# matteociccozzi/LayoutDiT

Hardware: AMD Instinct MI355X
Metric: images/sec ViT-B/16 224px bs=64 fwd (higher is better)
Workload: dtype f32; 1 GPU; ViT-base/16 224x224 bs=64 f32 forward, taps [4, 6, 8, 12] (BASELINE.json configs[1]); images_per_gpu=64, global_batch=64, parallelism=dp1: batch-sharded replicas, no data-path collective, weights=synthetic seed 0, images=synthetic doc-like pages, seed 1234, rank0_placement=128 CPUs: NUMA node 1 of GPU 0000:a4:00.0

## Files before the change

layoutdit_amd/csrc/attention_f32.hip:

```cpp
#include "ldit_common.h"

#ifdef LDIT_GEMM_STAMPS
__device__ unsigned long long *g_attn32_stamps = nullptr;
#define A32_STAMP(var) const unsigned long long var = __builtin_amdgcn_s_memtime()
#else
#define A32_STAMP(var)
#endif

namespace ldit {

namespace {

constexpr int KSTR = 68;
constexpr int VSTR = 64;

template <int KT, int NW>
__global__ void __launch_bounds__(NW * 64, NW == 4 ? 2 : NW / 4) attention_f32(const float *__restrict__ Q, const float *__restrict__ K,
                                                     const float *__restrict__ V, float *__restrict__ O, int N, int H,
                                                     int ldq, int ldk, int ldv, int ldo, float scale, int nqg)
{
    constexpr int KROWS = KT * 32;
    extern __shared__ __attribute__((aligned(16))) char smem[];
    float *Ks = reinterpret_cast<float *>(smem);
    float *Vs = Ks + KROWS * KSTR;

    const int tid = threadIdx.x, lane = tid & 63;
    const int wave = __builtin_amdgcn_readfirstlane(tid >> 6);
    const int li = lane & 31, lh = lane >> 5;
    const int bid = blockIdx.x;
    const int qg = bid % nqg, bh = bid / nqg, head = bh % H, b = bh / H;
    const int qt = qg * NW + wave;
    const bool active = qt * 32 < N;
    const size_t tok0 = (size_t)b * N;
#ifdef LDIT_GEMM_STAMPS
    unsigned long long ph[4] = {0, 0, 0, 0};
#endif
    A32_STAMP(t_begin);

    float q[32];
    {
        int qrow = qt * 32 + li;
        qrow = qrow < N ? qrow : N - 1;
        const f32x4 *qp = reinterpret_cast<const f32x4 *>(Q + (tok0 + qrow) * ldq + head * 64 + 32 * lh);
#pragma unroll
        for (int u = 0; u < 8; ++u) {
            const f32x4 t = qp[u];
            q[4 * u + 0] = t[0]; q[4 * u + 1] = t[1]; q[4 * u + 2] = t[2]; q[4 * u + 3] = t[3];
        }
    }

    f32x16 o[2];
#pragma unroll
    for (int e = 0; e < 16; ++e) { o[0][e] = 0.0f; o[1][e] = 0.0f; }
    float m_run = -INFINITY, l_run = 0.0f;

    for (int c0 = 0; c0 < N; c0 += KROWS) {
        const int nkeys = (N - c0) < KROWS ? (N - c0) : KROWS;
        const int ktiles = (nkeys + 31) >> 5;
        A32_STAMP(t0);
        if (c0) __syncthreads();
        {
            constexpr int PER = (32 * 16) / (NW * 64) > 0 ? (32 * 16) / (NW * 64) : 1;
            static_assert((32 * 16) % (NW * 64) == 0, "a key tile must split evenly over the threads");
            constexpr int BATCH = 4;
#pragma unroll
            for (int e = 0; e < PER; ++e)
#pragma unroll
                for (int k0 = 0; k0 < KT; k0 += BATCH) {
                    f32x4 kv[BATCH], vv[BATCH];
#pragma unroll
                    for (int i = 0; i < BATCH; ++i) {
                        const int kt = k0 + i, u = kt * 512 + e * NW * 64 + tid, row = u >> 4, c4 = (u & 15) * 4;
                        kv[i] = f32x4{0.f, 0.f, 0.f, 0.f};
                        vv[i] = f32x4{0.f, 0.f, 0.f, 0.f};
                        if (kt < KT && kt < ktiles && row < nkeys) {
                            kv[i] = *reinterpret_cast<const f32x4 *>(K + (tok0 + c0 + row) * ldk + head * 64 + c4);
                            vv[i] = *reinterpret_cast<const f32x4 *>(V + (tok0 + c0 + row) * ldv + head * 64 + c4);
                        }
                    }
#pragma unroll
                    for (int i = 0; i < BATCH; ++i) {
                        const int kt = k0 + i, u = kt * 512 + e * NW * 64 + tid, row = u >> 4, c4 = (u & 15) * 4;
                        if (kt < KT && kt < ktiles) {
                            *reinterpret_cast<f32x4 *>(Ks + row * KSTR + c4) = kv[i];
                            *reinterpret_cast<f32x4 *>(Vs + row * VSTR + c4) = vv[i];
                        }
                    }
                }
        }
        __syncthreads();
        if (!active) continue;
        A32_STAMP(t1);

        f32x16 s[KT];
#pragma unroll
        for (int kt = 0; kt < KT; ++kt) {
#pragma unroll
            for (int e = 0; e < 16; ++e) s[kt][e] = 0.0f;
            if (kt < ktiles) {
                const float *kr = Ks + (kt * 32 + li) * KSTR + 32 * lh;
#pragma unroll
                for (int u = 0; u < 8; ++u) {
                    const f32x4 kf = *reinterpret_cast<const f32x4 *>(kr + 4 * u);
#pragma unroll
                    for (int e = 0; e < 4; ++e)
                        s[kt] = __builtin_amdgcn_mfma_f32_32x32x2f32(kf[e], q[4 * u + e], s[kt], 0, 0, 0);
                }
            }
        }
#ifdef LDIT_GEMM_STAMPS
        asm volatile("s_nop 0" ::"v"(s[0][0]), "v"(s[KT - 1][0]));
#endif
        A32_STAMP(t2);
        float mx = -INFINITY;
#pragma unroll
        for (int kt = 0; kt < KT; ++kt) {
            if (kt < ktiles) {
                const bool partial = (kt + 1) * 32 > nkeys;
#pragma unroll
                for (int r = 0; r < 16; ++r) {
                    float v = s[kt][r] * scale;
                    if (partial && (kt * 32 + 8 * (r >> 2) + 4 * lh + (r & 3)) >= nkeys) v = -INFINITY;
                    s[kt][r] = v;
                    mx = fmaxf(mx, v);
                }
            }
        }
        mx = fmaxf(mx, __shfl_xor(mx, 32, 64));
        const float m_new = fmaxf(m_run, mx);
        const float alpha = __expf(m_run - m_new);
        m_run = m_new;
        float lsum = 0.0f;
#pragma unroll
        for (int kt = 0; kt < KT; ++kt) {
            if (kt < ktiles) {
#pragma unroll
                for (int r = 0; r < 16; ++r) {
                    const float pv = __expf(s[kt][r] - m_new);
                    s[kt][r] = pv;
                    lsum += pv;
                }
            }
        }
        l_run = l_run * alpha + lsum;
        if (c0) {
#pragma unroll
            for (int e = 0; e < 16; ++e) { o[0][e] *= alpha; o[1][e] *= alpha; }
        }
        A32_STAMP(t3);
#pragma unroll
        for (int kt = 0; kt < KT; ++kt) {
            if (kt < ktiles) {
                const int left = nkeys - kt * 32;
#pragma unroll
                for (int r = 0; r < 16; ++r) {
                    if (8 * (r >> 2) + (r & 3) >= left) continue;
                    const float *vr = Vs + (kt * 32 + 8 * (r >> 2) + 4 * lh + (r & 3)) * VSTR + li;
                    o[0] = __builtin_amdgcn_mfma_f32_32x32x2f32(vr[0], s[kt][r], o[0], 0, 0, 0);
                    o[1] = __builtin_amdgcn_mfma_f32_32x32x2f32(vr[32], s[kt][r], o[1], 0, 0, 0);
                }
            }
        }
#ifdef LDIT_GEMM_STAMPS
        asm volatile("s_nop 0" ::"v"(o[0][0]), "v"(o[1][0]));
        ph[0] += t1 - t0 + (c0 ? 0 : t0 - t_begin); ph[1] += t2 - t1; ph[2] += t3 - t2; ph[3] += __builtin_amdgcn_s_memtime() - t3;
#endif
    }

    if (!active) return;
#ifdef LDIT_GEMM_STAMPS
    if (g_attn32_stamps && wave == 0 && lane == 0) {
        unsigned long long *d = g_attn32_stamps + (size_t)blockIdx.x * 6;
        d[0] = ph[0]; d[1] = ph[1]; d[2] = ph[2]; d[3] = ph[3]; d[5] = __builtin_amdgcn_s_memtime() - t_begin;
    }
#endif
    const float l = l_run + __shfl_xor(l_run, 32, 64);
    const float inv = 1.0f / l;
    const int qrow = qt * 32 + li;
    if (qrow < N) {
        float *op = O + (tok0 + qrow) * ldo + head * 64 + 4 * lh;
#pragma unroll
        for (int dt = 0; dt < 2; ++dt)
#pragma unroll
            for (int g = 0; g < 4; ++g) {
                f32x4 t = {o[dt][4 * g + 0] * inv, o[dt][4 * g + 1] * inv, o[dt][4 * g + 2] * inv, o[dt][4 * g + 3] * inv};
                *reinterpret_cast<f32x4 *>(op + dt * 32 + 8 * g) = t;
            }
    }
}

}

int launch_attention(const float *Q, const float *K, const float *V, float *O, int B, int N, int H, int D, int ldq,
                     int ldk, int ldv, int ldo, float scale, hipStream_t stream)
{
    if (B <= 0 || N <= 0 || H <= 0) return fail(LDIT_EINVAL, "attention: empty problem");
    if (D != 64) return fail(LDIT_EUNSUPPORTED, "attention: head_dim=%d, only 64 is implemented", D);
    if (!Q || !K || !V || !O) return fail(LDIT_EINVAL, "attention: null operand");
    if ((ldq | ldk | ldv | ldo) & 3) return fail(LDIT_EINVAL, "attention: row strides must be multiples of 4 floats");
    if (!aligned16(Q) || !aligned16(K) || !aligned16(V) || !aligned16(O)) return fail(LDIT_EINVAL, "attention: operands must be 16-byte aligned");
    constexpr int KT = 7;
    constexpr int lds = KT * 32 * (KSTR + VSTR) * 4;
    const int nqt = (N + 31) / 32;
    auto go = [&](auto kern, int nw, std::atomic<unsigned long long> &attr_done) -> int {
        if (int rc = ensure_dynamic_lds(reinterpret_cast<const void *>(kern), lds, attr_done)) return rc;
        const int nqg = (nqt + nw - 1) / nw;
        hipLaunchKernelGGL(kern, dim3((unsigned)(B * H * nqg)), dim3(nw * 64), lds, stream, Q, K, V, O, N, H, ldq, ldk, ldv, ldo,
                           scale, nqg);
        LDIT_HIP_CHECK(hipGetLastError());
        return LDIT_OK;
    };
    static std::atomic<unsigned long long> set8{0}, set4{0};
    const long wgs8 = (long)B * H * ((nqt + 7) / 8);
    if (wgs8 <= 128 && nqt > 4) { if (int rc = go(attention_f32<KT, 4>, 4, set4)) return rc; }
    else if (int rc = go(attention_f32<KT, 8>, 8, set8)) return rc;
    LDIT_HIP_CHECK(hipGetLastError());
    return LDIT_OK;
}

}

#ifdef LDIT_GEMM_STAMPS
extern "C" int ldit_dbg_set_attn32_stamps(void *buf)
{
    unsigned long long *p = static_cast<unsigned long long *>(buf);
    return hipMemcpyToSymbol(HIP_SYMBOL(g_attn32_stamps), &p, sizeof(p)) == hipSuccess ? 0 : -3;
}
#endif
```

Baseline: 3432 images/sec.

## Use direct global-to-LDS loads and a persistent pipelined walk in f32 attention

Replaces the register-staged K/V copy into LDS with global_load_lds_dwordx4 direct-to-LDS DMA, using an XOR-swizzled K layout in place of the padded stride. When the whole sequence fits one key chunk (N <= 224, which holds for ViT-B/16's 197 tokens), it launches a persistent grid of one workgroup per CU. Each workgroup walks (image, head, query-group) items and prefetches the next item's K and Q while computing the current S and PV. The goal is to hide global load latency and cut VGPR traffic and launch tail. The cost is inline asm that manipulates m0, more complex barrier ordering, and fewer resident workgroups per CU.

```diff
diff --git a/layoutdit_amd/csrc/attention_f32.hip b/layoutdit_amd/csrc/attention_f32.hip
--- a/layoutdit_amd/csrc/attention_f32.hip
+++ b/layoutdit_amd/csrc/attention_f32.hip
@@ -11,34 +11,83 @@
 
 namespace {
 
-constexpr int KSTR = 68;
-constexpr int VSTR = 64;
-
-template <int KT, int NW>
+constexpr int ROWB = 256;
+
+__device__ __forceinline__ void glds16_sbase(const void *ubase, unsigned voff_bytes, unsigned lds_dst)
+{
+    unsigned keep;
+    asm volatile("s_mov_b32 %0, m0\n\ts_mov_b32 m0, %3\n\ts_nop 0\n\tglobal_load_lds_dwordx4 %1, %2\n\ts_mov_b32 m0, %0"
+                 : "=&s"(keep)
+                 : "v"(voff_bytes), "s"(ubase), "s"(lds_dst)
+                 : "memory");
+}
+
+__device__ __forceinline__ void dma_wait_and_barrier()
+{
+    asm volatile("s_waitcnt vmcnt(0)" ::: "memory");
+    __builtin_amdgcn_s_barrier();
+    asm volatile("" ::: "memory");
+}
+
+template <int KT, int NW, bool WALK>
 __global__ void __launch_bounds__(NW * 64, NW == 4 ? 2 : NW / 4) attention_f32(const float *__restrict__ Q, const float *__restrict__ K,
                                                      const float *__restrict__ V, float *__restrict__ O, int N, int H,
-                                                     int ldq, int ldk, int ldv, int ldo, float scale, int nqg)
-{
-    constexpr int KROWS = KT * 32;
+                                                     int ldq, int ldk, int ldv, int ldo, float scale, int nqg, int nitems)
+{
+    constexpr int KROWS = KT * 32, HALF = KROWS * ROWB;
+    constexpr int PPT = 8 / NW;
+    static_assert(8 % NW == 0, "the 8 pieces of a key tile must split evenly over the waves");
     extern __shared__ __attribute__((aligned(16))) char smem[];
-    float *Ks = reinterpret_cast<float *>(smem);
-    float *Vs = Ks + KROWS * KSTR;
+    const char *Ks = smem;
+    const float *Vs = reinterpret_cast<const float *>(smem + HALF);
+    const unsigned lds0 = __builtin_amdgcn_readfirstlane((unsigned)(uintptr_t)((__attribute__((address_space(3))) char *)smem));
 
     const int tid = threadIdx.x, lane = tid & 63;
     const int wave = __builtin_amdgcn_readfirstlane(tid >> 6);
     const int li = lane & 31, lh = lane >> 5;
-    const int bid = blockIdx.x;
-    const int qg = bid % nqg, bh = bid / nqg, head = bh % H, b = bh / H;
-    const int qt = qg * NW + wave;
-    const bool active = qt * 32 < N;
-    const size_t tok0 = (size_t)b * N;
-#ifdef LDIT_GEMM_STAMPS
-    unsigned long long ph[4] = {0, 0, 0, 0};
-#endif
-    A32_STAMP(t_begin);
+
+    const int p16 = lane & 15;
+    int rt[PPT];
+    unsigned koff[PPT], voff[PPT];
+#pragma unroll
+    for (int j = 0; j < PPT; ++j) {
+        rt[j] = 4 * (wave + NW * j) + (lane >> 4);
+        koff[j] = (unsigned)rt[j] * (unsigned)ldk * 4u + 16u * (unsigned)(p16 ^ (rt[j] & 15));
+        voff[j] = (unsigned)rt[j] * (unsigned)ldv * 4u + 16u * (unsigned)p16;
+    }
+    auto issue_k = [&](const float *kc, int nkeys) {
+#pragma unroll
+        for (int kt = 0; kt < KT; ++kt) {
+            const int left = nkeys - kt * 32;
+            if (left > 0) {
+                const unsigned toff = (unsigned)(kt * 32) * (unsigned)ldk * 4u;
+#pragma unroll
+                for (int j = 0; j < PPT; ++j) {
+                    unsigned off = koff[j];
+                    if (left < 32) off = (unsigned)(rt[j] < left ? rt[j] : left - 1) * (unsigned)ldk * 4u + 16u * (unsigned)(p16 ^ (rt[j] & 15));
+                    glds16_sbase(kc, off + toff, lds0 + (unsigned)((kt * 32 + 4 * (wave + NW * j)) * ROWB));
+                }
+            }
+        }
+    };
+    auto issue_v = [&](const float *vc, int nkeys) {
+#pragma unroll
+        for (int kt = 0; kt < KT; ++kt) {
+            const int left = nkeys - kt * 32;
+            if (left > 0) {
+                const unsigned toff = (unsigned)(kt * 32) * (unsigned)ldv * 4u;
+#pragma unroll
+                for (int j = 0; j < PPT; ++j) {
+                    unsigned off = voff[j];
+                    if (left < 32) off = (unsigned)(rt[j] < left ? rt[j] : left - 1) * (unsigned)ldv * 4u + 16u * (unsigned)p16;
+                    glds16_sbase(vc, off + toff, lds0 + (unsigned)(HALF + (kt * 32 + 4 * (wave + NW * j)) * ROWB));
+                }
+            }
+        }
+    };
 
     float q[32];
-    {
+    auto load_q = [&](size_t tok0, int head, int qt) {
         int qrow = qt * 32 + li;
         qrow = qrow < N ? qrow : N - 1;
         const f32x4 *qp = reinterpret_cast<const f32x4 *>(Q + (tok0 + qrow) * ldq + head * 64 + 32 * lh);
@@ -47,61 +96,31 @@
             const f32x4 t = qp[u];
             q[4 * u + 0] = t[0]; q[4 * u + 1] = t[1]; q[4 * u + 2] = t[2]; q[4 * u + 3] = t[3];
         }
-    }
-
-    f32x16 o[2];
-#pragma unroll
-    for (int e = 0; e < 16; ++e) { o[0][e] = 0.0f; o[1][e] = 0.0f; }
-    float m_run = -INFINITY, l_run = 0.0f;
-
-    for (int c0 = 0; c0 < N; c0 += KROWS) {
-        const int nkeys = (N - c0) < KROWS ? (N - c0) : KROWS;
-        const int ktiles = (nkeys + 31) >> 5;
-        A32_STAMP(t0);
-        if (c0) __syncthreads();
-        {
-            constexpr int PER = (32 * 16) / (NW * 64) > 0 ? (32 * 16) / (NW * 64) : 1;
-            static_assert((32 * 16) % (NW * 64) == 0, "a key tile must split evenly over the threads");
-            constexpr int BATCH = 4;
-#pragma unroll
-            for (int e = 0; e < PER; ++e)
-#pragma unroll
-                for (int k0 = 0; k0 < KT; k0 += BATCH) {
-                    f32x4 kv[BATCH], vv[BATCH];
-#pragma unroll
-                    for (int i = 0; i < BATCH; ++i) {
-                        const int kt = k0 + i, u = kt * 512 + e * NW * 64 + tid, row = u >> 4, c4 = (u & 15) * 4;
-                        kv[i] = f32x4{0.f, 0.f, 0.f, 0.f};
-                        vv[i] = f32x4{0.f, 0.f, 0.f, 0.f};
-                        if (kt < KT && kt < ktiles && row < nkeys) {
-                            kv[i] = *reinterpret_cast<const f32x4 *>(K + (tok0 + c0 + row) * ldk + head * 64 + c4);
-                            vv[i] = *reinterpret_cast<const f32x4 *>(V + (tok0 + c0 + row) * ldv + head * 64 + c4);
-                        }
-                    }
-#pragma unroll
-                    for (int i = 0; i < BATCH; ++i) {
-                        const int kt = k0 + i, u = kt * 512 + e * NW * 64 + tid, row = u >> 4, c4 = (u & 15) * 4;
-                        if (kt < KT && kt < ktiles) {
-                            *reinterpret_cast<f32x4 *>(Ks + row * KSTR + c4) = kv[i];
-                            *reinterpret_cast<f32x4 *>(Vs + row * VSTR + c4) = vv[i];
-                        }
-                    }
-                }
-        }
-        __syncthreads();
-        if (!active) continue;
-        A32_STAMP(t1);
-
-        f32x16 s[KT];
+    };
+    auto retire_q = [&]() {
+#pragma unroll
+        for (int j = 0; j < 32; ++j) asm volatile("" : "+v"(q[j]));
+    };
+
+    f32x16 s[KT], o[2];
+    float m_run, l_run;
+    auto reset_o = [&]() {
+#pragma unroll
+        for (int e = 0; e < 16; ++e) { o[0][e] = 0.0f; o[1][e] = 0.0f; }
+        m_run = -INFINITY; l_run = 0.0f;
+    };
+
+    const int kread = li * ROWB + ((8 * lh) ^ (li & 15)) * 16;
+    auto phase_s = [&](int ktiles) {
 #pragma unroll
         for (int kt = 0; kt < KT; ++kt) {
 #pragma unroll
             for (int e = 0; e < 16; ++e) s[kt][e] = 0.0f;
             if (kt < ktiles) {
-                const float *kr = Ks + (kt * 32 + li) * KSTR + 32 * lh;
+                const char *kr = Ks + kt * 32 * ROWB;
 #pragma unroll
                 for (int u = 0; u < 8; ++u) {
-                    const f32x4 kf = *reinterpret_cast<const f32x4 *>(kr + 4 * u);
+                    const f32x4 kf = *reinterpret_cast<const f32x4 *>(kr + (kread ^ (u * 16)));
 #pragma unroll
                     for (int e = 0; e < 4; ++e)
                         s[kt] = __builtin_amdgcn_mfma_f32_32x32x2f32(kf[e], q[4 * u + e], s[kt], 0, 0, 0);
@@ -111,7 +130,8 @@
 #ifdef LDIT_GEMM_STAMPS
         asm volatile("s_nop 0" ::"v"(s[0][0]), "v"(s[KT - 1][0]));
 #endif
-        A32_STAMP(t2);
+    };
+    auto phase_softmax = [&](int nkeys, int ktiles, bool rescale) {
         float mx = -INFINITY;
 #pragma unroll
         for (int kt = 0; kt < KT; ++kt) {
@@ -143,11 +163,12 @@
             }
         }
         l_run = l_run * alpha + lsum;
-        if (c0) {
+        if (rescale) {
 #pragma unroll
             for (int e = 0; e < 16; ++e) { o[0][e] *= alpha; o[1][e] *= alpha; }
         }
-        A32_STAMP(t3);
+    };
+    auto phase_pv = [&](int nkeys, int ktiles) {
 #pragma unroll
         for (int kt = 0; kt < KT; ++kt) {
             if (kt < ktiles) {
@@ -155,7 +176,7 @@
 #pragma unroll
                 for (int r = 0; r < 16; ++r) {
                     if (8 * (r >> 2) + (r & 3) >= left) continue;
-                    const float *vr = Vs + (kt * 32 + 8 * (r >> 2) + 4 * lh + (r & 3)) * VSTR + li;
+                    const float *vr = Vs + (kt * 32 + 8 * (r >> 2) + 4 * lh + (r & 3)) * 64 + li;
                     o[0] = __builtin_amdgcn_mfma_f32_32x32x2f32(vr[0], s[kt][r], o[0], 0, 0, 0);
                     o[1] = __builtin_amdgcn_mfma_f32_32x32x2f32(vr[32], s[kt][r], o[1], 0, 0, 0);
                 }
@@ -163,29 +184,116 @@
         }
 #ifdef LDIT_GEMM_STAMPS
         asm volatile("s_nop 0" ::"v"(o[0][0]), "v"(o[1][0]));
-        ph[0] += t1 - t0 + (c0 ? 0 : t0 - t_begin); ph[1] += t2 - t1; ph[2] += t3 - t2; ph[3] += __builtin_amdgcn_s_memtime() - t3;
-#endif
-    }
-
-    if (!active) return;
-#ifdef LDIT_GEMM_STAMPS
-    if (g_attn32_stamps && wave == 0 && lane == 0) {
-        unsigned long long *d = g_attn32_stamps + (size_t)blockIdx.x * 6;
-        d[0] = ph[0]; d[1] = ph[1]; d[2] = ph[2]; d[3] = ph[3]; d[5] = __builtin_amdgcn_s_memtime() - t_begin;
-    }
-#endif
-    const float l = l_run + __shfl_xor(l_run, 32, 64);
-    const float inv = 1.0f / l;
-    const int qrow = qt * 32 + li;
-    if (qrow < N) {
-        float *op = O + (tok0 + qrow) * ldo + head * 64 + 4 * lh;
-#pragma unroll
-        for (int dt = 0; dt < 2; ++dt)
-#pragma unroll
-            for (int g = 0; g < 4; ++g) {
-                f32x4 t = {o[dt][4 * g + 0] * inv, o[dt][4 * g + 1] * inv, o[dt][4 * g + 2] * inv, o[dt][4 * g + 3] * inv};
-                *reinterpret_cast<f32x4 *>(op + dt * 32 + 8 * g) = t;
-            }
+#endif
+    };
+    auto store_o = [&](size_t tok0, int head, int qt) {
+        const float l = l_run + __shfl_xor(l_run, 32, 64);
+        const float inv = 1.0f / l;
+        const int qrow = qt * 32 + li;
+        if (qrow < N) {
+            float *op = O + (tok0 + qrow) * ldo + head * 64 + 4 * lh;
+#pragma unroll
+            for (int dt = 0; dt < 2; ++dt)
+#pragma unroll
+                for (int g = 0; g < 4; ++g) {
+                    f32x4 t = {o[dt][4 * g + 0] * inv, o[dt][4 * g + 1] * inv, o[dt][4 * g + 2] * inv, o[dt][4 * g + 3] * inv};
+                    *reinterpret_cast<f32x4 *>(op + dt * 32 + 8 * g) = t;
+                }
+        }
+    };
+
+    int item = blockIdx.x;
+    int qg = item % nqg, bh = item / nqg, head = bh % H;
+    size_t tok0 = (size_t)(bh / H) * N;
+    int qt = qg * NW + wave;
+    bool active = qt * 32 < N;
+
+    if constexpr (WALK) {
+        const int step = gridDim.x;
+#ifdef LDIT_GEMM_STAMPS
+        unsigned long long ordinal = 1;
+#endif
+        issue_k(K + tok0 * ldk + head * 64, N);
+        load_q(tok0, head, qt);
+        for (;;) {
+            int n = N;
+            asm volatile("" : "+s"(n));
+            const int ktiles = (n + 31) >> 5;
+            A32_STAMP(t0);
+            retire_q();
+            dma_wait_and_barrier();
+            A32_STAMP(t1);
+            issue_v(V + tok0 * ldv + head * 64, n);
+            if (active) phase_s(ktiles);
+            const int next = item + step;
+            const bool more = next < nitems;
+            const int nqg_ = next % nqg, nbh = next / nqg, nhead = nbh % H;
+            const size_t ntok0 = (size_t)(nbh / H) * N;
+            const int nqt = nqg_ * NW + wave;
+            if (more) load_q(ntok0, nhead, nqt);
+            A32_STAMP(t2);
+            if (active) { reset_o(); phase_softmax(n, ktiles, false); }
+            A32_STAMP(t3);
+            retire_q();
+            dma_wait_and_barrier();
+            A32_STAMP(t4);
+            if (more) issue_k(K + ntok0 * ldk + nhead * 64, n);
+            if (active) phase_pv(n, ktiles);
+            A32_STAMP(t5);
+            if (active) store_o(tok0, head, qt);
+#ifdef LDIT_GEMM_STAMPS
+            if (g_attn32_stamps && active && wave == 0 && lane == 0) {
+                unsigned long long *d = g_attn32_stamps + (size_t)item * 8;
+                const unsigned long long t6 = __builtin_amdgcn_s_memtime();
+                d[0] = t1 - t0; d[1] = t2 - t1; d[2] = t3 - t2; d[3] = t4 - t3; d[4] = t5 - t4; d[5] = t6 - t5; d[6] = t6 - t0;
+                d[7] = ordinal;
+            }
+            ++ordinal;
+#endif
+            if (!more) break;
+            item = next; head = nhead; tok0 = ntok0; qt = nqt;
+            active = qt * 32 < N;
+        }
+    } else {
+#ifdef LDIT_GEMM_STAMPS
+        unsigned long long ph[4] = {0, 0, 0, 0};
+#endif
+        A32_STAMP(t_begin);
+        load_q(tok0, head, qt);
+        retire_q();
+        reset_o();
+        for (int c0 = 0; c0 < N; c0 += KROWS) {
+            const int nkeys = (N - c0) < KROWS ? (N - c0) : KROWS;
+            const int ktiles = (nkeys + 31) >> 5;
+            A32_STAMP(t0);
+            if (c0) {
+                __builtin_amdgcn_s_barrier();
+                asm volatile("" ::: "memory");
+            }
+            issue_k(K + (tok0 + c0) * ldk + head * 64, nkeys);
+            issue_v(V + (tok0 + c0) * ldv + head * 64, nkeys);
+            dma_wait_and_barrier();
+            if (!active) continue;
+            A32_STAMP(t1);
+            phase_s(ktiles);
+            A32_STAMP(t2);
+            phase_softmax(nkeys, ktiles, c0 != 0);
+            A32_STAMP(t3);
+            phase_pv(nkeys, ktiles);
+#ifdef LDIT_GEMM_STAMPS
+            ph[0] += t1 - t0 + (c0 ? 0 : t0 - t_begin); ph[1] += t2 - t1; ph[2] += t3 - t2; ph[3] += __builtin_amdgcn_s_memtime() - t3;
+#endif
+        }
+        if (!active) return;
+        A32_STAMP(t_store);
+        store_o(tok0, head, qt);
+#ifdef LDIT_GEMM_STAMPS
+        if (g_attn32_stamps && wave == 0 && lane == 0) {
+            unsigned long long *d = g_attn32_stamps + (size_t)item * 8;
+            const unsigned long long t_end = __builtin_amdgcn_s_memtime();
+            d[0] = ph[0]; d[1] = ph[1]; d[2] = ph[2]; d[3] = 0; d[4] = ph[3]; d[5] = t_end - t_store; d[6] = t_end - t_begin; d[7] = 1;
+        }
+#endif
     }
 }
 
@@ -200,22 +308,32 @@
     if ((ldq | ldk | ldv | ldo) & 3) return fail(LDIT_EINVAL, "attention: row strides must be multiples of 4 floats");
     if (!aligned16(Q) || !aligned16(K) || !aligned16(V) || !aligned16(O)) return fail(LDIT_EINVAL, "attention: operands must be 16-byte aligned");
     constexpr int KT = 7;
-    constexpr int lds = KT * 32 * (KSTR + VSTR) * 4;
+    constexpr int lds = 2 * KT * 32 * ROWB;
     const int nqt = (N + 31) / 32;
+    const bool walk = N <= KT * 32;
     auto go = [&](auto kern, int nw, std::atomic<unsigned long long> &attr_done) -> int {
         if (int rc = ensure_dynamic_lds(reinterpret_cast<const void *>(kern), lds, attr_done)) return rc;
         const int nqg = (nqt + nw - 1) / nw;
-        hipLaunchKernelGGL(kern, dim3((unsigned)(B * H * nqg)), dim3(nw * 64), lds, stream, Q, K, V, O, N, H, ldq, ldk, ldv, ldo,
-                           scale, nqg);
+        const long items = (long)B * H * nqg;
+        if (items > 0x7fffffffL) return fail(LDIT_EINVAL, "attention: too many (image, head, query group) items");
+        long wgs = items;
+        if (walk) {
+            const int cus = compute_units();
+            if (cus <= 0) return fail(LDIT_EHIP, "attention: no compute units reported");
+            wgs = items < cus ? items : cus;
+        }
+        hipLaunchKernelGGL(kern, dim3((unsigned)wgs), dim3(nw * 64), lds, stream, Q, K, V, O, N, H, ldq, ldk, ldv, ldo, scale, nqg,
+                           (int)items);
         LDIT_HIP_CHECK(hipGetLastError());
         return LDIT_OK;
     };
-    static std::atomic<unsigned long long> set8{0}, set4{0};
+    static std::atomic<unsigned long long> set8w{0}, set4w{0}, set8{0}, set4{0};
     const long wgs8 = (long)B * H * ((nqt + 7) / 8);
-    if (wgs8 <= 128 && nqt > 4) { if (int rc = go(attention_f32<KT, 4>, 4, set4)) return rc; }
-    else if (int rc = go(attention_f32<KT, 8>, 8, set8)) return rc;
-    LDIT_HIP_CHECK(hipGetLastError());
-    return LDIT_OK;
+    const bool four = wgs8 <= 128 && nqt > 4;
+    int rc;
+    if (walk) rc = four ? go(attention_f32<KT, 4, true>, 4, set4w) : go(attention_f32<KT, 8, true>, 8, set8w);
+    else rc = four ? go(attention_f32<KT, 4, false>, 4, set4) : go(attention_f32<KT, 8, false>, 8, set8);
+    return rc;
 }
 
 }
```

New measurement: 3450 images/sec, median of 6. Within noise of the previous version (+0.5%).
